# brson/synth2

Measured on AMD Instinct MI355X. Metric: voice-samples/sec (mono) at 64k voices per GPU, 48 kHz, 1024-frame buffers, higher is better.
Workload: dtype f32

## Files before the change

include/s2r.h:

```cpp
#ifndef S2R_H
#define S2R_H
#include <stddef.h>
#include <stdint.h>

#ifdef __cplusplus
extern "C" {
#endif

#define S2R_ABI_VERSION 4

typedef enum {
    S2R_OK = 0,
    S2R_ERR_INVALID = -1,
    S2R_ERR_NO_DEVICE = -2,
    S2R_ERR_HIP = -3,
    S2R_ERR_PATCH_SYNTAX = -4,
    S2R_ERR_PATCH_RANGE = -5,
    S2R_ERR_TOO_MANY_FRAMES = -6,
    S2R_ERR_OFFSET_OVERFLOW = -7,
    S2R_ERR_OUT_OF_MEMORY = -8
} s2r_status;

typedef enum { S2R_OSC_SQUARE = 0, S2R_OSC_SAW = 1, S2R_OSC_TRIANGLE = 2, S2R_OSC_SINE = 3,
               S2R_OSC_DPW_SAW = 4, S2R_OSC_DPW_SQUARE = 5, S2R_OSC_DPW_TRIANGLE = 6 } s2r_osc_kind;
// ... 189 lines not shown
uint32_t s2r_shard_voices(const s2r_synth *s);
uint32_t s2r_block_voices(const s2r_synth *s);
uint32_t s2r_device_count(const s2r_synth *s);
uint64_t s2r_double_release_count(const s2r_synth *s);
int s2r_set_low_latency(s2r_synth *s, int enabled);
int s2r_low_latency_active(const s2r_synth *s);
#define S2R_EXCHANGE_HANDLE_BYTES 64
int s2r_exchange_create(s2r_synth *s, uint32_t n_ranks, void *handle_out, size_t handle_bytes);
int s2r_exchange_attach(s2r_synth *s, uint32_t rank, uint32_t n_ranks, const void *handle, size_t handle_bytes);
int s2r_set_resident(s2r_synth *s, int enabled);
int s2r_resident_active(const s2r_synth *s);
int s2r_quiesce(s2r_synth *s);
int s2r_set_timing(s2r_synth *s, int enabled);
int s2r_set_flat_shortcut(s2r_synth *s, int enabled);
int s2r_set_coeff_stream(s2r_synth *s, int enabled);
float s2r_last_render_ms(s2r_synth *s);
const char *s2r_last_error(const s2r_synth *s);
const char *s2r_status_string(int status);


#define S2R_STREAM_CHARS_PER_SAMPLE 18u
#define S2R_STREAM_FRAMES 4096u
#define S2R_STREAM_RATE_HZ 32000u
size_t s2r_stream_frame_json(const float *samples, size_t n, char *out, size_t cap);

int s2r_parse_patch_text(const char *text, size_t len, s2r_patch *out, char *err_buf, size_t err_cap);

float s2r_voice_pan(float pan, float key_spread, uint8_t note);
void s2r_pan_gains(float p, float *gl, float *gr);

// ... 22 lines not shown
```

synth2_amd/csrc/s2r_device.h:

```cpp
#pragma once
#include <hip/hip_runtime_api.h>
#include <stdint.h>
#include "s2r.h"

#define S2R_VF_STARTED 1u
#define S2R_VF_RELEASED 2u

struct S2rEnv {
    float A;
    float D;
    float S;
    float R;
    float sus_off;
    float slope_att;
    float slope_dec;
    float slope_rel;
};

struct S2rVoiceArrays {
    float *pitch;
    uint32_t *offset;
    uint32_t *release;
    uint32_t *flags;
    float *phase;
// ... 81 lines not shown
    uint32_t super_frames;
    S2rVoiceArrays v;
    float *block_partials;
    float *direct_out;
    int32_t direct_stereo;
    S2rDone done;
    float *per_voice;
    const float *sin_table;
    const float *noise_tab;
    S2rTabRef tab;
    const S2rTimedEvent *tev;
    int32_t *voice_ev_head;
    unsigned long long *stamps;
    unsigned long long *timeline;
    uint32_t tl_slot;
    const S2rBankEntry *bank;
    uint32_t bank_size;
    const uint32_t *ov_heads_counter;
    uint32_t ov_heads_target;
    uint32_t *ov_render_counter;
    uint32_t *ov_fail;
    const S2rTimedEvent *tev_src;
    S2rTimedEvent *tev_copy;
    const uint32_t *slices;
    uint32_t *arrive;
    uint32_t arrive_target;
    S2rMixTail mt;
};

struct S2rVoiceEvent {
    uint32_t voice;
    uint32_t flags;
    float pitch;
    uint32_t seed;
};
#define S2R_EV_RESTART 1u
#define S2R_EV_RELEASE 2u
#define S2R_EV_PROGRAM_SHIFT 16

struct S2rTimedEvent {
    uint32_t voice;
    uint32_t frame;
    uint32_t flags;
// ... 198 lines not shown
```

synth2_amd/csrc/s2r_host.cpp:

```cpp
#include <hip/hip_runtime.h>
#include <algorithm>
#include <cmath>
#include <cstdarg>
#include <cstdio>
#include <cstdlib>
#include <cstring>
#include <ctime>
#include <atomic>
#include <memory>
#include <new>
#include <string>
#include <vector>

#include "s2r.h"
#include "s2r_device.h"
#include "s2r_math.h"
#include "s2r_patch.h"
#include "s2r_post.h"
#include "s2r_rules.h"
#include "s2r_voices.h"

namespace {

constexpr int kEventSlots = 4;
// ... 218 lines not shown
    float *pan_partials = nullptr;
    std::vector<hipEvent_t> pan_ev;
    size_t pan_ev_used = 0;
    float pan_mix_ms = -1.0f;
    char *bus_gains_host = nullptr, *bus_gains_dev = nullptr;
    hipEvent_t bus_gains_sent = nullptr;
    float *bus_partials = nullptr;
    float *bus_out = nullptr, *bus_out_dev = nullptr;
    float bus_mix_ms = -1.0f;
    bool bus_dev_ramped = false;
    S2rPostChain post;
    float pitch_table[256];
    hipEvent_t t0 = nullptr, t1 = nullptr;
    bool timing = false, timed = false, no_flat_shortcut = false;
    uint64_t double_release = 0;
    s2r_voice_log_fn voice_log = nullptr;
    void *voice_log_user = nullptr;
    bool broken = false;
    std::string err = "";
};


namespace {

int set_err(s2r_synth *s, int code, const char *fmt, ...) {
    if (s) {
        char buf[512];
        va_list ap; va_start(ap, fmt); vsnprintf(buf, sizeof buf, fmt, ap); va_end(ap);
        s->err = buf;
    }
// ... 293 lines not shown
    p.sr = (float)sample_rate;
    p.rcp_sr = 1.0f / p.sr;
    p.fast_div_sr = (fast_div_rate(sample_rate) && s->bank[0].lpf_freq >= 0x1p-30f && s->bank[0].lpf_freq <= 0x1p30f) ? 1 : 0;
    p.no_flat_shortcut = s->no_flat_shortcut ? 1 : 0;
    p.frames = (uint32_t)frames;
    p.n_voices = s->shard_voices;
    p.frames_stride = partials_stride(s->cfg.max_frames);
    p.v = s->v;
    p.block_partials = s->block_partials;
    p.per_voice = nullptr;
    p.sin_table = s->sin_dev;
    { static const bool off = [] { const char *e = std::getenv("S2R_NOISE_TAB"); return e && e[0] == '0'; }();
      p.noise_tab = off ? nullptr : s->noise_dev; }
    p.bank = s->bank_dev;
    p.bank_size = (uint32_t)s->bank.size();
    return p;
}

int ensure_bank(s2r_synth *s, uint32_t sample_rate, hipStream_t stream, bool *bank_kernel_out) {
    bool bank_kernel = s->bank.size() > 1;
    for (const s2r_patch &pt : s->bank) if (pt.osc_kind > S2R_OSC_SINE) bank_kernel = true;
    if (bank_kernel && (s->bank_dirty || s->bank_rate != sample_rate)) {
        std::vector<S2rBankEntry> host(s->bank.size());
        std::vector<S2rTabBuild> builds(s->bank.size());
        size_t tab_floats = 0;
        const float srf = (float)sample_rate;
        for (size_t k = 0; k < s->bank.size(); k++) {
            const s2r_patch &pt = s->bank[k];
            S2rBankEntry &e = host[k];
            std::memset(&e, 0, sizeof e);
// ... 1048 lines not shown
    if (s->voice_mem) (void)hipFree(s->voice_mem);
    if (s->bank_dev) (void)hipFree(s->bank_dev);
    if (s->os_buf) (void)hipFree(s->os_buf);
    if (s->os_taps) (void)hipFree(s->os_taps);
    if (s->block_partials) (void)hipFree(s->block_partials);
    if (s->out_dev) (void)hipFree(s->out_dev);
    if (s->out_host) (void)hipHostFree(s->out_host);
    if (s->done_host) (void)hipHostFree(s->done_host);
    if (s->done_counter) (void)hipFree(s->done_counter);
    for (int k = 0; k < 2; k++) {
        if (s->ring_host[k]) (void)hipHostFree(s->ring_host[k]);
        if (s->ring_done[k]) (void)hipEventDestroy(s->ring_done[k]);
    }
    if (s->sin_dev) (void)hipFree(s->sin_dev);
    if (s->noise_dev) (void)hipFree(s->noise_dev);
    if (s->res_cmd_vram && s->res_cmd) (void)hipFree(s->res_cmd);
    if (s->res_host) (void)hipHostFree(s->res_host);
    if (s->res_gran) (void)hipHostFree(s->res_gran);
    if (s->per_voice_dev) (void)hipFree(s->per_voice_dev);
    if (s->gains_host) (void)hipHostFree(s->gains_host);
    if (s->gains_dev) (void)hipFree(s->gains_dev);
    if (s->gains_sent) (void)hipEventDestroy(s->gains_sent);
    if (s->pan_rows) (void)hipFree(s->pan_rows);
    if (s->pan_partials) (void)hipFree(s->pan_partials);
    if (s->bus_gains_host) (void)hipHostFree(s->bus_gains_host);
    if (s->bus_gains_dev) (void)hipFree(s->bus_gains_dev);
    if (s->bus_gains_sent) (void)hipEventDestroy(s->bus_gains_sent);
    if (s->bus_partials) (void)hipFree(s->bus_partials);
    if (s->bus_out) (void)hipHostFree(s->bus_out);
    s->post.release();
// ... 183 lines not shown
    }
    CREATE_HIP(hipEventCreate(&s->t0));
    CREATE_HIP(hipEventCreate(&s->t1));
    {
        float table[1024];
        build_sin_table(table);
        if (crc32_bytes(table, sizeof table) != kSinTableCrc) {
            fprintf(stderr, "libs2r: regenerated SIN_TABLE does not match the reference table (CRC mismatch)\n");
            release_all(s);
            return S2R_ERR_INVALID;
        }
        CREATE_HIP(hipMalloc((void **)&s->sin_dev, sizeof table));
        CREATE_HIP(hipMemcpy(s->sin_dev, table, sizeof table, hipMemcpyHostToDevice));
        CREATE_HIP(hipMalloc((void **)&s->noise_dev, 65536 * sizeof(float)));
        CREATE_HIP(s2r_launch_noise_table(s->noise_dev, s->stream));
    }
    CREATE_HIP(hipStreamSynchronize(s->stream));
#undef CREATE_HIP
    *out = s;
    return S2R_OK;
}


int s2r_create(const s2r_config *cfg, s2r_synth **out) {
    if (!cfg || !out || cfg->struct_size != sizeof(s2r_config)) return S2R_ERR_INVALID;
    *out = nullptr;
    if (cfg->n_devices <= 1) {
        s2r_config one = *cfg;
        if (cfg->n_devices == 1) one.device = cfg->devices[0];
        one.n_devices = 0;
// ... 1038 lines not shown
}

uint32_t s2r_shard_voices(const s2r_synth *s) { return s ? s->shard_voices : 0; }
uint32_t s2r_block_voices(const s2r_synth *s) { return s ? s->block_voices : 0; }
uint32_t s2r_device_count(const s2r_synth *s) { return s ? (s->kids.empty() ? 1u : (uint32_t)s->kids.size()) : 0; }
uint64_t s2r_double_release_count(const s2r_synth *s) { return s ? s->double_release : 0; }

int s2r_set_flat_shortcut(s2r_synth *s, int enabled) {
    if (!s) return S2R_ERR_INVALID;
    S2R_QUIESCE(s);
    s->no_flat_shortcut = enabled == 0;
    for (s2r_synth *kid : s->kids) kid->no_flat_shortcut = s->no_flat_shortcut;
    return S2R_OK;
}

int s2r_set_coeff_stream(s2r_synth *s, int enabled) {
    if (!s) return S2R_ERR_INVALID;
    S2R_QUIESCE(s);
    s->use_tab = enabled != 0;
    s->use_arg_events = enabled != 2 && enabled != 4;
    s->bank_dirty = true;
    for (s2r_synth *kid : s->kids) { kid->use_tab = s->use_tab; kid->use_arg_events = s->use_arg_events; kid->bank_dirty = true; }
    return S2R_OK;
}

int s2r_set_low_latency(s2r_synth *s, int enabled) {
    if (!s) return S2R_ERR_INVALID;
    if (s->parent || !s->kids.empty()) return set_err(s, S2R_ERR_INVALID, "s2r_set_low_latency takes a single-device handle");
    S2R_QUIESCE(s);
    if (enabled && !s->res_host) {
// ... 211 lines not shown
```

synth2_amd/csrc/s2r_kern_common.h:

```cpp
#pragma once
#include <hip/hip_runtime.h>
#include <type_traits>
#include "s2r_device.h"
#include "s2r_math.h"

namespace {

__constant__ uint64_t c_exp2f_table[S2R_EXP2F_N] = S2R_EXP2F_TABLE_INIT;

constexpr int kChunk = 16;
constexpr uint32_t kSuperMax = 256;
constexpr uint32_t kSuperWhole = 1024;
constexpr int kP = 4;
constexpr uint32_t kTileRow = 68;

typedef float f4 __attribute__((ext_vector_type(4)));
typedef int i4 __attribute__((ext_vector_type(4)));
typedef unsigned u4 __attribute__((ext_vector_type(4)));
typedef unsigned short us4 __attribute__((ext_vector_type(4)));
typedef double d4 __attribute__((ext_vector_type(4)));
typedef unsigned long long ul4 __attribute__((ext_vector_type(4)));

__device__ __forceinline__ f4 vfma(f4 a, f4 b, f4 c) { return __builtin_elementwise_fma(a, b, c); }
__device__ __forceinline__ d4 vfma(d4 a, d4 b, d4 c) { return __builtin_elementwise_fma(a, b, c); }
// ... 703 lines not shown
        out[j] = __builtin_fmaf((s2 - s1) / 1.0f, s.tv[j] - (float)s.i1[j], s1);
    }
    return out;
}
template <bool FMV>
__device__ __forceinline__ f4 sine_quad(f4 x, f4 period, double rcp_period, const float *sSin) {
    SineQuad s = sine_quad_issue<FMV>(x, period, rcp_period, sSin);
    return sine_quad_finish(s);
}

typedef float fp2 __attribute__((ext_vector_type(2)));
__device__ __forceinline__ f4 pk_add4(f4 a, f4 b) {
    fp2 lo, hi;
    asm("v_pk_add_f32 %0, %1, %2" : "=v"(lo) : "v"(a.xy), "v"(b.xy));
    asm("v_pk_add_f32 %0, %1, %2" : "=v"(hi) : "v"(a.zw), "v"(b.zw));
    return (f4){lo.x, lo.y, hi.x, hi.y};
}

__device__ __forceinline__ void combine_groups(const S2rRenderParams &p, const S2rDone &done, const float *sWbuf, uint32_t n_groups, uint32_t super_frames,
                                               uint32_t n_sc, uint32_t sc0, float *bp_sc, uint32_t tid, uint32_t n_threads,
                                               unsigned long long *granules = nullptr, uint32_t granule_tag = 0u, bool wt = false) {
    for (uint32_t f = 4u * tid; f < n_sc; f += 4u * n_threads) {
        const float *row = sWbuf + f;
        f4 acc;
        {
            const f4 v0 = *reinterpret_cast<const f4 *>(row), v1 = *reinterpret_cast<const f4 *>(row + super_frames),
                     v2 = *reinterpret_cast<const f4 *>(row + 2u * super_frames), v3 = *reinterpret_cast<const f4 *>(row + 3u * super_frames);
            acc = pk_add4(pk_add4(pk_add4(v0, v1), v2), v3);
        }
        for (uint32_t g = 4u; g < n_groups; g += 4u) {
// ... 291 lines not shown
            ctl.mt.final_done = S2rDone{pl.final_flag + sel, s_cmd[3], nullptr};
            ctl.mt.final_stereo = stereo;
        } else {
            ctl.mt.out = o;
            ctl.mt.stereo = stereo;
            ctl.mt.done = S2rDone{pl.done_flag + sel, s_cmd[3], pl.done_counter + sel};
            if (s_cmd[12] != 0u && pl.granules != nullptr) { ctl.mt.granules = pl.granules; ctl.mt.granule_tag = s_cmd[3]; }
        }
        }
        if (frames != 0u && frames <= a.p.frames) fill(ctl);
        __syncthreads();
    }
    if (blockIdx.x == 0u && tid == 0u) __hip_atomic_store(pl.exited, pl.launch_id, __ATOMIC_RELAXED, __HIP_MEMORY_SCOPE_SYSTEM);
}

template <int OSC, int SRC, int FILT = 0, bool FMV = false, int NZ = 0, bool AFLAT = false>
__device__ __forceinline__ void chunk_fast(const S2rRenderParams &p, VoiceRegs &r, const EnvRun &ea, const EnvRun &em,
                                           const FlatCache &fc, const OscK &k, uint32_t o_chunk, const float *tab,
                                           const uint64_t *sT, const float *sSin, bool live, uint32_t tile_m0,
                                           float *pv_dst, const FiltCoef *fcoef = nullptr, Filt2 *f2 = nullptr) {
    constexpr bool SMALL = NZ >= 1, ALIGNED = NZ == 2;
    tile_set_base(tile_m0);
    f4 xq[4], bq[4], gq[4], pq[4], iq[4];
    if (SRC == 1) {
        const uint32_t plane = p.tab.plane;
#pragma unroll
        for (int q = 0; q < 4; ++q) {
            xq[q] = load_f4u(tab + 4 * q);
            if (FILT != 0) { bq[q] = load_f4u(tab + plane + 4 * q); gq[q] = load_f4u(tab + 2u * plane + 4 * q); }
            if (FMV) pq[q] = load_f4u(tab + p.tab.fm_plane * plane + 4 * q);
        }
    }
    const double rcp_period = (OSC == S2R_OSC_SINE && !FMV) ? s2r_rcp_f64(k.period) : 0.0;
    r.last = live ? r.last : 0.0f;
    const float ea_slope = live ? ea.s0 : 0.0f, ea_base = live ? ea.s1 : 0.0f, ea_y0 = live ? ea.s2 : 0.0f;
    const float xc0 = live ? fc.xc : 1.0f;
    f4 amp[4], nz[4];
    const float t_chunk = (float)o_chunk;
    const uint32_t o_lo = o_chunk & 0xffffu;
    uint32_t o01 = pk_add_u16(o_lo | (o_lo << 16), 0x00010000u), o23 = pk_add_u16(o01, 0x00020002u);
    const uint32_t seed_pair = (r.seed_rot & 0xffffu) | (r.seed_rot << 16);
    f4 t_small = splat(t_chunk) + (f4){0.0f, 1.0f, 2.0f, 3.0f};
    f4 nzt[4];
    if (ALIGNED) {
        const float *np = p.noise_tab + ((r.seed_rot ^ o_chunk) & 0xffffu);
#pragma unroll
        for (int q = 0; q < 4; ++q) nzt[q] = *reinterpret_cast<const f4 *>(np + 4 * q);
    }
#pragma unroll
    for (int q = 0; q < 4; ++q) {
        f4 t;
        if (ALIGNED) {
            t = t_small;
            t_small = t_small + splat(4.0f);
            nz[q] = nzt[q];
        } else if (SMALL) {
            t = t_small;
            nz[q] = hash_noise4_low16(seed_pair, o01, o23);
            t_small = t_small + splat(4.0f);
            o01 = pk_add_u16(o01, 0x00040004u); o23 = pk_add_u16(o23, 0x00040004u);
        } else {
            const u4 ou = (u4)(o_chunk + 4u * q) + (u4){0u, 1u, 2u, 3u};
            t = __builtin_convertvector(ou, f4);
            nz[q] = hash_noise4(r.seed_rot, t) + splat(p.noise_level);
        }
        if (AFLAT) amp[q] = splat(ea_slope * (t_chunk - ea_base) + ea_y0);
        else amp[q] = splat(ea_slope) * pk_add4(t, splat(-ea_base)) + splat(ea_y0);
// ... 3 lines not shown
            pq[q] = splat(p.sr) / f_osc;
            iq[q] = splat(1.0f) / pq[q];
        }
        if (SRC == 2) {
            const f4 mod = splat(em.s0) * (t - splat(em.s1)) + splat(em.s2);
            const f4 f_lpf = pow2_sleef_core4(mod * splat(p.amt_lpf)) * splat(p.lpf_freq);
            const f4 num = splat(-2.0f * 3.14159274101257324f) * f_lpf;
            const f4 arg = p.fast_div_sr ? div_const_nocheck4(num, p.sr, p.rcp_sr) : (num / splat(p.sr));
            xq[q] = expf4(arg, sT);
        }
    }
    const uint32_t livemask = live ? 0xffffffffu : 0u;
    f4 outs[4];
#pragma unroll
    for (int q = 0; q < 4; ++q) {
        f4 a0 = splat(1.0f) - xq[q];
        if (SRC == 2 && !live) a0 = splat(0.0f);
        const f4 period = FMV ? pq[q] : splat(k.period), inv_period = FMV ? iq[q] : splat(k.inv_period);
        f4 ph;
        float phc = r.phase;
#pragma unroll
        for (int j = 0; j < 4; ++j) {
            ph[j] = phc;
            phc = __builtin_amdgcn_fractf(phc + inv_period[j]);
        }
        r.phase = phc;
        const f4 x = period * ph;
        f4 osc;
        if (OSC == S2R_OSC_SAW) {
            const f4 ka = FMV ? splat(-2.0f) * inv_period : splat(k.a);
            osc = vfma(ka, x, splat(1.0f));
// ... 22 lines not shown
                if (SRC == 1) { cj.alpha = xq[q][j]; cj.beta = bq[q][j]; cj.gamma = gq[q][j]; }
                y[j] = dsp_filter_apply(FILT, cj, sv[j], *f2);
            }
        }
        f4 out = y * amp[q];
        if (FILT != 0) out = (f4)((u4)out & livemask);
        tile_store4(q, out);
        outs[q] = out;
    }
    if (pv_dst) {
#pragma unroll
        for (int q = 0; q < 4; ++q) *reinterpret_cast<f4u *>(pv_dst + 4 * q) = outs[q];
    }
}

}
```

synth2_amd/csrc/s2r_render_onepole.inc:

```
#include "s2r_kern_common.h"

namespace {

template <int OSC, bool FM, int MODE, int MAXT>
__device__ __forceinline__ void render_fill(const S2rRenderArgs &a, const FillCtl &ctl) {
    const S2rRenderParams &p = a.p;
    constexpr bool PV = MODE == 1;
    constexpr bool TEV = MODE == 2;
    const uint32_t kSuper = p.super_frames;
    __shared__ uint64_t sT[S2R_EXP2F_N];
    __shared__ __attribute__((aligned(8))) float sSin[OSC == S2R_OSC_SINE ? 2048 : 2];
    extern __shared__ __attribute__((aligned(16))) float s_dyn[];
    __shared__ uint32_t s_word;

    const uint32_t tid = threadIdx.x;
    const uint32_t lane = tid & 63u, wave = tid >> 6, n_waves = blockDim.x >> 6;
    constexpr uint32_t VW = 64;
    constexpr uint32_t GW = VW / 16;
    const uint32_t n_groups = n_waves * GW;
    float *const sW = s_dyn;
    constexpr uint32_t kTile = kChunk * kTileRow;
    const uint32_t sw_floats = s2r_sw_buffers(p.frames, kSuper) * n_groups * kSuper;
    float *const tile = s_dyn + sw_floats + wave * kTile;
    float *const wave_scratch = s_dyn + sw_floats + n_waves * kTile + wave * 64u;
    const uint32_t tile_lds = (uint32_t)__builtin_amdgcn_readfirstlane((int)(uint32_t)(uintptr_t)tile);
    const uint32_t vi = blockIdx.x * blockDim.x + tid;
#if defined(S2R_STAMPS)
    uint32_t stamp_k = 0;
    auto stamp = [&](uint32_t slot) { if (p.stamps && lane == 0 && slot < 16u) p.stamps[(size_t)(vi >> 6) * 16u + slot] = __builtin_amdgcn_s_memtime(); };
    stamp(0);
#else
    auto stamp = [&](uint32_t) {};
    uint32_t stamp_k = 0; (void)stamp_k;
#endif
    uint32_t dbg_events = 0, dbg_dense = 0, dbg_general = 0, dbg_runs = 0, dbg_runchunks = 0;
    unsigned long long dbg_t_dense = 0, dbg_t_run = 0;
    unsigned long long dbg_t_top = 0, dbg_t_sel = 0; (void)dbg_t_top; (void)dbg_t_sel;
    unsigned long long dbg_t_pick1 = 0, dbg_t_casc = 0; (void)dbg_t_pick1; (void)dbg_t_casc;
    (void)dbg_events; (void)dbg_dense; (void)dbg_general; (void)dbg_runs; (void)dbg_runchunks; (void)dbg_t_dense; (void)dbg_t_run;
// ... 116 lines not shown
    uint32_t buf = 0;

    auto reduce_chunk = [&](uint32_t f_base, uint32_t n_frames) {
        const uint32_t f = lane & 15u, grp = lane >> 4;
        __builtin_amdgcn_wave_barrier();
        if (f < n_frames) {
            const float *src = tile + f * kTileRow + grp * 16u;
            float acc = src[0];
#pragma unroll
            for (int k = 1; k < 16; ++k) acc += src[k];
            sW[(buf * n_groups + wave * GW + grp) * kSuper + f_base + f] = acc;
        }
        __builtin_amdgcn_wave_barrier();
    };

    bool w_flat = false, w_aflat = false, w_aligned = false, w_small = false;
    auto reclassify_stages = [&]() {
        w_flat = !p.no_flat_shortcut && __ballot(live && em.s0 != 0.0f) == 0ull &&
                 (!FM || __ballot(!(fc.k.period >= 0x1p-126f && fc.k.period < __builtin_inff())) == 0ull);
        w_aflat = __ballot(live && ea.s0 != 0.0f) == 0ull;
    };
    auto reclassify = [&]() {
        reclassify_stages();
        w_aligned = p.noise_tab != nullptr && __ballot(((r.offset | r.seed_rot) & 15u) != 0u) == 0ull;
        w_small = __ballot(r.offset + ctl.frames > (1u << 24)) == 0ull;
    };
    reclassify();
    stamp(1);

    auto apply_events_lane = [&](uint32_t fpos) -> bool {
        bool restarted = false, released_now = false;
        took_release = false;
        while (ev_frame == fpos) {
            const S2rTimedEvent e = ev_next;
            if (e.flags & S2R_EV_RESTART) {
// ... 48 lines not shown
    };

    auto apply_events_at = [&](uint32_t fpos) {
        if (!wave_events || __ballot(ev_frame == fpos) == 0ull) return;
        dbg_events += (uint32_t)__builtin_popcountll(__ballot(ev_frame == fpos));
        bool restarted = false;
        if (ev_frame == fpos) restarted = apply_events_lane(fpos);
        if (__ballot(restarted) != 0ull) {
            w_aligned = p.noise_tab != nullptr && __ballot(((r.offset | r.seed_rot) & 15u) != 0u) == 0ull;
            w_small = __ballot(r.offset + ctl.frames > (1u << 24)) == 0ull;
        }
        wave_events = __ballot(ev_idx >= 0) != 0ull;
        w_flat = !p.no_flat_shortcut && __ballot(live && em.s0 != 0.0f) == 0ull &&
                 (!FM || __ballot(!(fc.k.period >= 0x1p-126f && fc.k.period < __builtin_inff())) == 0ull);
        w_aflat = __ballot(live && ea.s0 != 0.0f) == 0ull;
    };

    auto end_of_release = [&](float t0) {
        if (ea.s4 == 3.0f && !(t0 < ea.s3)) { ea.s0 = 0.0f; ea.s1 = 0.0f; ea.s2 = 0.0f; ea.s3 = __builtin_inff(); ea.s4 = 4.0f; }
        if (em.s4 == 3.0f && !(t0 < em.s3)) { em.s0 = 0.0f; em.s1 = 0.0f; em.s2 = 0.0f; em.s3 = __builtin_inff(); em.s4 = 4.0f; }
        if (ea.s4 == 2.0f && !(t0 < ea.s3)) { const bool rel = t0 < r.end_a;
            ea.s0 = rel ? p.amp.slope_rel : 0.0f; ea.s1 = rel ? r.ro_a : 0.0f; ea.s2 = rel ? p.amp.S : 0.0f;
            ea.s3 = rel ? r.end_a : __builtin_inff(); ea.s4 = rel ? 3.0f : 4.0f; }
        if (em.s4 == 2.0f && !(t0 < em.s3)) { const bool rel = t0 < r.end_m;
            em.s0 = rel ? p.mod.slope_rel : 0.0f; em.s1 = rel ? r.ro_m : 0.0f; em.s2 = rel ? p.mod.S : 0.0f;
            em.s3 = rel ? r.end_m : __builtin_inff(); em.s4 = rel ? 3.0f : 4.0f; }
    };

    const uint32_t rf = lane & 15u, rgrp = lane >> 4;
    const float *const tsrc = tile + rf * kTileRow + rgrp * 16u;
// ... 153 lines not shown
                    bool flat = false, tab_ok = false, offs_small = false;
                    if (run) {
                        run = (uint32_t)__builtin_amdgcn_readfirstlane((int)run);
                        offs_small = w_small || __ballot(o_chunk + run * kChunk > (1u << 24)) == 0ull;
                        flat = w_flat;
                        tab_ok = !flat && have_tab && offs_small;
                        if (FM && !flat && !tab_ok) run = 0;
                        if (FM && !flat && __ballot(live && !(p.sr >= r.pitch * 0x1p-115f)) != 0ull) run = 0;
                    }
                    if (run) {
                        ++dbg_runs; dbg_runchunks += run;
                        const unsigned long long dbg_tr0 = S2R_DBG_NOW();
                        dbg_t_sel += dbg_tr0 - dbg_ts0;
                        float *const sw_row = sW + (buf * n_groups + wave * GW + rgrp) * kSuper + rf;
                        const TabCur cur = tab_cursor(p.tab, em.s4, r.ro_m > p.mod.sus_off, r.release_u, live);
                        auto run_chunks = [&](auto src_tag, auto nz_tag, auto aflat_tag) {
                            constexpr int SRC = decltype(src_tag)::value;
                            constexpr int NZ = decltype(nz_tag)::value;
                            constexpr bool AFLAT = decltype(aflat_tag)::value;
                            for (uint32_t i = 0; i < run; ++i) {
                                const uint32_t f0 = c16 + i * kChunk;
                                *pend_dst = tsum();
                                float *pvd = (PV && in_range) ? p.per_voice + pv_base + sc0 + f0 : nullptr;
                                const uint32_t oc = o_chunk + i * kChunk;
                                const float *tp = p.tab.base + (ptrdiff_t)(cur.idx + (int32_t)(oc & cur.mask));
                                chunk_fast<OSC, SRC, 0, (FM && SRC == 1), NZ, AFLAT>(p, r, ea, em, fc, FM ? fc.k : k_const, oc, tp, sT, sSin, live,
                                                                              tile_lds, pvd);
                                __builtin_amdgcn_wave_barrier();
                                pend_dst = sw_row + f0;
                            }
                        };
                        const bool small = p.noise_level == 0.0f && offs_small;
                        const bool aligned = small && w_aligned && ((sc0 + c16) & 15u) == 0u;
                        const bool aflat = aligned && w_aflat;
                        using T = std::true_type; using F = std::false_type;
                        using N0 = std::integral_constant<int, 0>; using N1 = std::integral_constant<int, 1>; using N2 = std::integral_constant<int, 2>;
                        if (tab_ok) {
                            if (aflat) run_chunks(N1{}, N2{}, T{});
                            else if (aligned) run_chunks(N1{}, N2{}, F{});
                            else if (small) run_chunks(N1{}, N1{}, F{});
                            else run_chunks(N1{}, N0{}, F{});
                        } else if (flat) {
                            if (aflat) run_chunks(N0{}, N2{}, T{});
                            else if (aligned) run_chunks(N0{}, N2{}, F{});
                            else if (small) run_chunks(N0{}, N1{}, F{});
                            else run_chunks(N0{}, N0{}, F{});
                        } else if (!FM) {
                            if (aligned) run_chunks(N2{}, N2{}, F{});
                            else if (small) run_chunks(N2{}, N1{}, F{});
                            else run_chunks(N2{}, N0{}, F{});
                        }
                        c16 += (run - 1u) * kChunk;
                        dbg_t_run += S2R_DBG_NOW() - dbg_tr0;
                        continue;
                    }
                }
                flush_pending();
                ++dbg_general;
                for (uint32_t g = c16; g < c16 + kChunk; g += kP) {
                    FrameCF4 cf; OscK4 kf;
                    closed_form_x4<OSC, FM>(p, r, ea, em, thr_min, fc, fcc, r.offset + sc0 + g, sT, cf, kf);
                    f4 out4;
#pragma unroll
                    for (int j = 0; j < kP; ++j) {
                        FrameCF c1; c1.amp = cf.amp[j]; c1.xc = cf.xc[j]; c1.nz = cf.nz[j];
// ... 42 lines not shown
        p.v.offset[vi] = (!ev_dirty && o > 0xffffffffu - ctl.frames) ? 0xffffffffu : o + ctl.frames;
        p.v.phase[vi] = r.phase;
        p.v.lpf_last[vi] = r.last;
        if (ev_dirty) {
            p.v.pitch[vi] = r.pitch;
            p.v.release[vi] = r.release_u;
            p.v.flags[vi] = S2R_VF_STARTED | (r.released ? S2R_VF_RELEASED : 0u);
            p.v.seed[vi] = seed_now;
            if (ev_restart) {
                p.v.fx1[vi] = 0.0f; p.v.fx2[vi] = 0.0f; p.v.fy1[vi] = 0.0f; p.v.fy2[vi] = 0.0f;
                p.v.osc_z[vi] = s2r_u2f(S2R_OSC_Z_NONE);
                p.v.program[vi] = program_now;
            }
        }
    }
    if (p.direct_out && ctl.granules == nullptr) signal_done(ctl.done, 1u);
    if (ctl.ov_render_counter != nullptr) ov_signal(ctl.ov_render_counter);
#if defined(S2R_STAMPS)
    if (p.stamps && lane == 0) p.stamps[(size_t)(vi >> 6) * 16u + 8u] = __builtin_amdgcn_s_memrealtime();
    if (ctl.fused) fused_tail(p, ctl, sW, &s_word, p.stamps ? p.stamps + (size_t)(vi >> 6) * 16u : nullptr);
#else
    if (ctl.fused) fused_tail(p, ctl, sW, &s_word);
#endif
#if defined(S2R_STAMPS)
    if (p.stamps && lane == 0) { unsigned long long *d = p.stamps + (size_t)(vi >> 6) * 16u; d[11] = dbg_events; d[12] = (unsigned long long)dbg_dense | ((dbg_t_pick1 & 0x3fffffull) << 20) | ((dbg_t_casc & 0x3fffffull) << 42); d[13] = (dbg_t_top << 32) | (dbg_t_sel & 0xffffffffull); d[14] = dbg_runs;
        d[10] = ((unsigned long long)dbg_runchunks << 48) | ((dbg_t_dense & 0xffffffull) << 24) | (dbg_t_run & 0xffffffull); }
#endif
    stamp(15);
    tl_mark(p.timeline, p.tl_slot, 1);
}

template <int OSC, bool FM, int MODE, int MAXT>
__global__ void __launch_bounds__(MAXT, (MAXT == 256 ? 2 : 1)) s2r_render_kernel(const S2rRenderArgs a) {
    const FillCtl ctl = fill_ctl_from_args(a);
    render_fill<OSC, FM, MODE, MAXT>(a, ctl);
}

template <int OSC, bool FM>
__global__ void __launch_bounds__(256, 1) s2r_resident_kernel(const S2rRenderArgs a, const S2rResident rs) {
    __shared__ uint32_t s_cmd[S2R_RES_CMD_WORDS];
    const uint32_t tid = threadIdx.x, lane = tid & 63u;
    uint32_t last = rs.first_seq - 1u;
    for (;;) {
        if (tid < 64u) {
            const unsigned long long t0 = __builtin_amdgcn_s_memrealtime();
            uint32_t polls = 0;
            for (;;) {
                uint32_t w = 0u;
                if (lane < S2R_RES_CMD_WORDS) w = __hip_atomic_load(rs.cmd + lane, __ATOMIC_RELAXED, __HIP_MEMORY_SCOPE_SYSTEM);
                const uint32_t s_first = (uint32_t)__builtin_amdgcn_readlane((int)w, 0), s_last = (uint32_t)__builtin_amdgcn_readlane((int)w, 31);
// ... 26 lines not shown
}

template <int OSC, bool FM>
__global__ void __launch_bounds__(256, 1) s2r_pool_kernel(const S2rRenderArgs a, const S2rPool pl) {
    pool_loop(a, pl, [&](const FillCtl &ctl) __attribute__((always_inline)) { render_fill<OSC, FM, 2, 256>(a, ctl); });
}

template <int OSC, bool FM, int MODE>
hipError_t launch_mode(const S2rRenderArgs &a0, uint32_t block_voices, hipStream_t stream) {
    static thread_local S2rRenderArgs a;
    a = a0;
    S2rRenderParams &p = a.p;
    const uint32_t grid = (p.n_voices + block_voices - 1) / block_voices;
    const uint32_t n_waves = block_voices / 64, n_groups = n_waves * 4;
    p.super_frames = s2r_pick_super_frames(n_groups, grid, p.frames);
    const size_t lds = sizeof(float) * ((size_t)s2r_sw_buffers(p.frames, p.super_frames) * n_groups * p.super_frames + (size_t)n_waves * (kChunk * kTileRow + 64));
    if (lds > 65536) {
        static thread_local size_t told256 = 0, told1024 = 0;
        if (block_voices <= 256 && told256 < lds) {
            const hipError_t e = hipFuncSetAttribute((const void *)s2r_render_kernel<OSC, FM, MODE, 256>, hipFuncAttributeMaxDynamicSharedMemorySize, (int)lds);
            if (e != hipSuccess) return e;
            told256 = lds;
        } else if (block_voices > 256 && told1024 < lds) {
            const hipError_t e = hipFuncSetAttribute((const void *)s2r_render_kernel<OSC, FM, MODE, 1024>, hipFuncAttributeMaxDynamicSharedMemorySize, (int)lds);
            if (e != hipSuccess) return e;
            told1024 = lds;
        }
    }
    if (block_voices <= 256) hipLaunchKernelGGL((s2r_render_kernel<OSC, FM, MODE, 256>), dim3(grid), dim3(block_voices), lds, stream, a);
    else hipLaunchKernelGGL((s2r_render_kernel<OSC, FM, MODE, 1024>), dim3(grid), dim3(block_voices), lds, stream, a);
    return hipGetLastError();
}

template <int OSC, bool FM>
hipError_t launch_resident(const S2rRenderArgs &a0, const S2rResident &rs, uint32_t block_voices, hipStream_t stream) {
    static thread_local S2rRenderArgs a;
    a = a0;
    S2rRenderParams &p = a.p;
    if (block_voices > 256u || p.n_voices > block_voices || p.direct_out == nullptr || p.per_voice != nullptr || p.tev != nullptr) return hipErrorInvalidValue;
    const uint32_t n_waves = block_voices / 64, n_groups = n_waves * 4;
    p.super_frames = s2r_pick_super_frames(n_groups, 1u, p.frames);
    const size_t lds = sizeof(float) * ((size_t)s2r_sw_buffers(p.frames, p.super_frames) * n_groups * p.super_frames + (size_t)n_waves * (kChunk * kTileRow + 64));
    if (lds > 65536) {
        static thread_local size_t told = 0;
        if (told < lds) {
            const hipError_t e = hipFuncSetAttribute((const void *)s2r_resident_kernel<OSC, FM>, hipFuncAttributeMaxDynamicSharedMemorySize, (int)lds);
            if (e != hipSuccess) return e;
            told = lds;
        }
    }
    hipLaunchKernelGGL((s2r_resident_kernel<OSC, FM>), dim3(1), dim3(block_voices), lds, stream, a, rs);
    return hipGetLastError();
}

template <int OSC, bool FM>
hipError_t launch_pool(const S2rRenderArgs &a0, const S2rPool &pl, uint32_t block_voices, hipStream_t stream) {
    static thread_local S2rRenderArgs a;
    a = a0;
    S2rRenderParams &p = a.p;
    if (block_voices > 256u || p.per_voice != nullptr || p.direct_out != nullptr) return hipErrorInvalidValue;
    const uint32_t grid = (p.n_voices + block_voices - 1) / block_voices;
    const uint32_t n_waves = block_voices / 64, n_groups = n_waves * 4;
    p.super_frames = s2r_pick_super_frames(n_groups, grid, p.frames);
    const size_t lds = sizeof(float) * ((size_t)s2r_sw_buffers(p.frames, p.super_frames) * n_groups * p.super_frames + (size_t)n_waves * (kChunk * kTileRow + 64));
    if (lds > 65536) {
        static thread_local size_t told = 0;
        if (told < lds) {
            const hipError_t e = hipFuncSetAttribute((const void *)s2r_pool_kernel<OSC, FM>, hipFuncAttributeMaxDynamicSharedMemorySize, (int)lds);
            if (e != hipSuccess) return e;
            told = lds;
        }
    }
    hipLaunchKernelGGL((s2r_pool_kernel<OSC, FM>), dim3(grid), dim3(block_voices), lds, stream, a, pl);
    return hipGetLastError();
}

}

// ... 22 lines not shown
```

synth2_amd/synth.py:

```python
import ctypes as C
import os

import numpy as np

from . import build as _build

OSC_SQUARE, OSC_SAW, OSC_TRIANGLE, OSC_SINE = 0, 1, 2, 3
OSC_DPW_SAW, OSC_DPW_SQUARE, OSC_DPW_TRIANGLE = 4, 5, 6

S2R_OK = 0
S2R_ERR_INVALID = -1
S2R_ERR_NO_DEVICE = -2
S2R_ERR_HIP = -3
S2R_ERR_PATCH_SYNTAX = -4
S2R_ERR_PATCH_RANGE = -5
S2R_ERR_TOO_MANY_FRAMES = -6
S2R_ERR_OFFSET_OVERFLOW = -7
S2R_ERR_OUT_OF_MEMORY = -8
MAX_BUSES = 8
MAX_IR_TAPS = 65536
MAX_DELAY_FRAMES = 262144
IR_SEGMENT = 256
METER_BLOCK = 256
LIMITER_MAX_LOOKAHEAD = 1024
# ... 183 lines not shown
        "s2r_set_noise_seed": (C.c_int, [H, C.c_uint32, C.c_uint32]),
        "s2r_shard_voices": (C.c_uint32, [H]),
        "s2r_block_voices": (C.c_uint32, [H]),
        "s2r_device_count": (C.c_uint32, [H]),
        "s2r_double_release_count": (C.c_uint64, [H]),
        "s2r_set_timing": (C.c_int, [H, C.c_int]),
        "s2r_set_low_latency": (C.c_int, [H, C.c_int]),
        "s2r_low_latency_active": (C.c_int, [H]),
        "s2r_set_resident": (C.c_int, [H, C.c_int]),
        "s2r_resident_active": (C.c_int, [H]),
        "s2r_quiesce": (C.c_int, [H]),
        "s2r_exchange_create": (C.c_int, [H, C.c_uint32, C.c_void_p, C.c_size_t]),
        "s2r_exchange_attach": (C.c_int, [H, C.c_uint32, C.c_uint32, C.c_void_p, C.c_size_t]),
        "s2r_set_flat_shortcut": (C.c_int, [H, C.c_int]),
        "s2r_set_coeff_stream": (C.c_int, [H, C.c_int]),
        "s2r_last_render_ms": (C.c_float, [H]),
        "s2r_last_error": (C.c_char_p, [H]),
        "s2r_parse_patch_text": (C.c_int, [C.c_char_p, C.c_size_t, C.POINTER(Patch), C.c_char_p, C.c_size_t]),
        "s2r_voice_pool_create": (H, [C.c_uint32]),
        "s2r_voice_pool_destroy": (None, [H]),
        "s2r_voice_pool_note_on": (C.c_uint32, [H, C.c_uint8, C.c_float]),
        "s2r_voice_pool_note_off": (C.c_int64, [H, C.c_uint8]),
        "s2r_voice_pool_advance": (None, [H, C.c_uint64]),
        "s2r_voice_pool_next_voice": (C.c_uint32, [H]),
        "s2r_voice_pool_set_threads": (None, [H, C.c_uint32, C.c_size_t]),
        "s2r_voice_pool_resolve": (C.c_uint32, [H, C.c_void_p, C.c_size_t, C.c_uint32, C.c_void_p]),
        "s2r_voice_pool_query": (C.c_int, [H, C.c_uint32, C.POINTER(VoiceState)]),
    }
    for name, (res, args) in sig.items():
        if _build.AB_LIB and not hasattr(L, name):
# ... 524 lines not shown

    def import_state(self, arr):
        arr = np.ascontiguousarray(arr, dtype=VOICE_STATE_DTYPE)
        assert arr.size == self.shard_voices
        self._check(self.L.s2r_import_state(self.h, arr.ctypes.data))

    def set_noise_seed(self, voice_index, seed):
        self._check(self.L.s2r_set_noise_seed(self.h, voice_index, seed))

    def set_flat_shortcut(self, enabled=True):
        self._check(self.L.s2r_set_flat_shortcut(self.h, 1 if enabled else 0))

    def set_coeff_stream(self, enabled=True):
        self._check(self.L.s2r_set_coeff_stream(self.h, int(enabled)))

    def set_low_latency(self, enabled=True):
        self._check(self.L.s2r_set_low_latency(self.h, 1 if enabled else 0))

    @property
    def low_latency_active(self):
        return bool(self.L.s2r_low_latency_active(self.h))

    def set_resident(self, enabled=True):
        self._check(self.L.s2r_set_resident(self.h, 1 if enabled else 0))

    @property
    def resident_active(self):
        return bool(self.L.s2r_resident_active(self.h))

    def quiesce(self):
# ... 24 lines not shown
```

Baseline: 1652 billion.

## Share per-frame oscillator, envelope and noise window across wave-uniform voices

Adds a per-wave check for whether all 64 lanes share the same table cursor, offset, noise seed and envelope state. When they do, and the run is long enough, the lanes work together to compute the wavetable sample, 1-x, amplitude ramp and noise for the run once into an LDS window, and each lane's chunk then reads those planes. This removes per-lane redundant table, noise and envelope work. The cost is extra LDS per wave, which can lower occupancy, plus classification ballots and a global atomic counter. The path is on by default for 256-thread non-FM kernels.

New measurement: 1707 billion (median of 6 runs). 3.3% higher.

```diff
diff --git a/include/s2r.h b/include/s2r.h
--- a/include/s2r.h
+++ b/include/s2r.h
@@ -227,6 +227,8 @@
 int s2r_set_timing(s2r_synth *s, int enabled);
 int s2r_set_flat_shortcut(s2r_synth *s, int enabled);
 int s2r_set_coeff_stream(s2r_synth *s, int enabled);
+int s2r_set_uniform_window(s2r_synth *s, int enabled);
+int s2r_uniform_window_chunks(s2r_synth *s, uint64_t *chunks);
 float s2r_last_render_ms(s2r_synth *s);
 const char *s2r_last_error(const s2r_synth *s);
 const char *s2r_status_string(int status);
diff --git a/synth2_amd/csrc/s2r_device.h b/synth2_amd/csrc/s2r_device.h
--- a/synth2_amd/csrc/s2r_device.h
+++ b/synth2_amd/csrc/s2r_device.h
@@ -119,6 +119,7 @@
     unsigned long long *stamps;
     unsigned long long *timeline;
     uint32_t tl_slot;
+    uint32_t uw_frames;
     const S2rBankEntry *bank;
     uint32_t bank_size;
     const uint32_t *ov_heads_counter;
@@ -131,7 +132,11 @@
     uint32_t *arrive;
     uint32_t arrive_target;
     S2rMixTail mt;
-};
+    uint32_t *uw_count;
+};
+#define S2R_UW_FRAMES 1024u
+#define S2R_UW_PLANES 4u
+#define S2R_UW_MIN_RUN 3u
 
 struct S2rVoiceEvent {
     uint32_t voice;
diff --git a/synth2_amd/csrc/s2r_host.cpp b/synth2_amd/csrc/s2r_host.cpp
--- a/synth2_amd/csrc/s2r_host.cpp
+++ b/synth2_amd/csrc/s2r_host.cpp
@@ -256,6 +256,8 @@
     hipEvent_t t0 = nullptr, t1 = nullptr;
     bool timing = false, timed = false, no_flat_shortcut = false;
     uint64_t double_release = 0;
+    bool uniform_window = true;
+    uint32_t *uw_count_dev = nullptr;
     s2r_voice_log_fn voice_log = nullptr;
     void *voice_log_user = nullptr;
     bool broken = false;
@@ -579,6 +581,7 @@
       p.noise_tab = off ? nullptr : s->noise_dev; }
     p.bank = s->bank_dev;
     p.bank_size = (uint32_t)s->bank.size();
+    p.uw_count = s->uniform_window ? s->uw_count_dev : nullptr;
     return p;
 }
 
@@ -1657,6 +1660,7 @@
     }
     if (s->sin_dev) (void)hipFree(s->sin_dev);
     if (s->noise_dev) (void)hipFree(s->noise_dev);
+    if (s->uw_count_dev) (void)hipFree(s->uw_count_dev);
     if (s->res_cmd_vram && s->res_cmd) (void)hipFree(s->res_cmd);
     if (s->res_host) (void)hipHostFree(s->res_host);
     if (s->res_gran) (void)hipHostFree(s->res_gran);
@@ -1870,6 +1874,8 @@
         CREATE_HIP(hipMemcpy(s->sin_dev, table, sizeof table, hipMemcpyHostToDevice));
         CREATE_HIP(hipMalloc((void **)&s->noise_dev, 65536 * sizeof(float)));
         CREATE_HIP(s2r_launch_noise_table(s->noise_dev, s->stream));
+        CREATE_HIP(hipMalloc((void **)&s->uw_count_dev, sizeof(uint32_t)));
+        CREATE_HIP(hipMemsetAsync(s->uw_count_dev, 0, sizeof(uint32_t), s->stream));
     }
     CREATE_HIP(hipStreamSynchronize(s->stream));
 #undef CREATE_HIP
@@ -2938,6 +2944,33 @@
     return S2R_OK;
 }
 
+int s2r_set_uniform_window(s2r_synth *s, int enabled) {
+    if (!s) return S2R_ERR_INVALID;
+    S2R_QUIESCE(s);
+    s->uniform_window = enabled != 0;
+    for (s2r_synth *kid : s->kids) kid->uniform_window = s->uniform_window;
+    return S2R_OK;
+}
+
+int s2r_uniform_window_chunks(s2r_synth *s, uint64_t *chunks) {
+    if (!s || !chunks) return S2R_ERR_INVALID;
+    S2R_QUIESCE(s);
+    uint64_t total = 0;
+    auto one = [&](s2r_synth *h) -> int {
+        if (!h->uw_count_dev) return S2R_OK;
+        uint32_t n = 0;
+        S2R_HIP(s, hipSetDevice(h->device));
+        S2R_HIP(s, hipDeviceSynchronize());
+        S2R_HIP(s, hipMemcpy(&n, h->uw_count_dev, sizeof n, hipMemcpyDeviceToHost));
+        total += n;
+        return S2R_OK;
+    };
+    if (s->kids.empty()) { S2R_TRY(one(s)); }
+    else for (s2r_synth *kid : s->kids) { S2R_TRY(one(kid)); }
+    *chunks = total;
+    return S2R_OK;
+}
+
 int s2r_set_coeff_stream(s2r_synth *s, int enabled) {
     if (!s) return S2R_ERR_INVALID;
     S2R_QUIESCE(s);
diff --git a/synth2_amd/csrc/s2r_kern_common.h b/synth2_amd/csrc/s2r_kern_common.h
--- a/synth2_amd/csrc/s2r_kern_common.h
+++ b/synth2_amd/csrc/s2r_kern_common.h
@@ -741,6 +741,12 @@
     fp2 lo, hi;
     asm("v_pk_add_f32 %0, %1, %2" : "=v"(lo) : "v"(a.xy), "v"(b.xy));
     asm("v_pk_add_f32 %0, %1, %2" : "=v"(hi) : "v"(a.zw), "v"(b.zw));
+    return (f4){lo.x, lo.y, hi.x, hi.y};
+}
+__device__ __forceinline__ f4 pk_sub4(f4 a, f4 b) {
+    fp2 lo, hi;
+    asm("v_pk_add_f32 %0, %1, %2 neg_lo:[0,1] neg_hi:[0,1]" : "=v"(lo) : "v"(a.xy), "v"(b.xy));
+    asm("v_pk_add_f32 %0, %1, %2 neg_lo:[0,1] neg_hi:[0,1]" : "=v"(hi) : "v"(a.zw), "v"(b.zw));
     return (f4){lo.x, lo.y, hi.x, hi.y};
 }
 
@@ -1062,15 +1068,26 @@
     if (blockIdx.x == 0u && tid == 0u) __hip_atomic_store(pl.exited, pl.launch_id, __ATOMIC_RELAXED, __HIP_MEMORY_SCOPE_SYSTEM);
 }
 
-template <int OSC, int SRC, int FILT = 0, bool FMV = false, int NZ = 0, bool AFLAT = false>
+template <int OSC, int SRC, int FILT = 0, bool FMV = false, int NZ = 0, bool AFLAT = false, bool UW = false>
 __device__ __forceinline__ void chunk_fast(const S2rRenderParams &p, VoiceRegs &r, const EnvRun &ea, const EnvRun &em,
                                            const FlatCache &fc, const OscK &k, uint32_t o_chunk, const float *tab,
                                            const uint64_t *sT, const float *sSin, bool live, uint32_t tile_m0,
-                                           float *pv_dst, const FiltCoef *fcoef = nullptr, Filt2 *f2 = nullptr) {
+                                           float *pv_dst, const FiltCoef *fcoef = nullptr, Filt2 *f2 = nullptr,
+                                           const float *win = nullptr) {
     constexpr bool SMALL = NZ >= 1, ALIGNED = NZ == 2;
+    static_assert(!UW || (SRC == 1 && FILT == 0 && !FMV && NZ == 2 && !AFLAT), "the uniform window replaces one variant only");
     tile_set_base(tile_m0);
     f4 xq[4], bq[4], gq[4], pq[4], iq[4];
-    if (SRC == 1) {
+    f4 a0w[4], ampw[4], nzw[4];
+    if (UW) {
+#pragma unroll
+        for (int q = 0; q < 4; ++q) {
+            xq[q] = *reinterpret_cast<const f4 *>(win + 4 * q);
+            a0w[q] = *reinterpret_cast<const f4 *>(win + S2R_UW_FRAMES + 4 * q);
+            ampw[q] = *reinterpret_cast<const f4 *>(win + 2u * S2R_UW_FRAMES + 4 * q);
+            nzw[q] = *reinterpret_cast<const f4 *>(win + 3u * S2R_UW_FRAMES + 4 * q);
+        }
+    } else if (SRC == 1) {
         const uint32_t plane = p.tab.plane;
 #pragma unroll
         for (int q = 0; q < 4; ++q) {
@@ -1090,7 +1107,7 @@
     const uint32_t seed_pair = (r.seed_rot & 0xffffu) | (r.seed_rot << 16);
     f4 t_small = splat(t_chunk) + (f4){0.0f, 1.0f, 2.0f, 3.0f};
     f4 nzt[4];
-    if (ALIGNED) {
+    if (ALIGNED && !UW) {
         const float *np = p.noise_tab + ((r.seed_rot ^ o_chunk) & 0xffffu);
 #pragma unroll
         for (int q = 0; q < 4; ++q) nzt[q] = *reinterpret_cast<const f4 *>(np + 4 * q);
@@ -1098,7 +1115,10 @@
 #pragma unroll
     for (int q = 0; q < 4; ++q) {
         f4 t;
-        if (ALIGNED) {
+        if (UW) {
+            nz[q] = nzw[q]; amp[q] = ampw[q];
+            continue;
+        } else if (ALIGNED) {
             t = t_small;
             t_small = t_small + splat(4.0f);
             nz[q] = nzt[q];
@@ -1132,7 +1152,7 @@
     f4 outs[4];
 #pragma unroll
     for (int q = 0; q < 4; ++q) {
-        f4 a0 = splat(1.0f) - xq[q];
+        f4 a0 = UW ? a0w[q] : SRC == 1 ? pk_sub4(splat(1.0f), xq[q]) : splat(1.0f) - xq[q];
         if (SRC == 2 && !live) a0 = splat(0.0f);
         const f4 period = FMV ? pq[q] : splat(k.period), inv_period = FMV ? iq[q] : splat(k.inv_period);
         f4 ph;
@@ -1185,4 +1205,26 @@
     }
 }
 
-}
+__device__ __forceinline__ void uw_fill(const S2rRenderParams &p, const EnvRun &ea, uint32_t seed_rot, uint32_t o_run, uint32_t run,
+                                        const float *tab_run, float *win, uint32_t lane) {
+    const uint32_t n_quads = 4u * run;
+    for (uint32_t q0 = 0; q0 < n_quads; q0 += 64u) {
+        const uint32_t Q = q0 + lane;
+        if (Q < n_quads) {
+            const uint32_t o = o_run + 4u * Q;
+            const f4 x = load_f4u(tab_run + 4u * Q);
+            const f4 a0 = pk_sub4(splat(1.0f), x);
+            const f4 t = splat((float)o) + (f4){0.0f, 1.0f, 2.0f, 3.0f};
+            const f4 amp = splat(ea.s0) * pk_add4(t, splat(-ea.s1)) + splat(ea.s2);
+            const f4 nz = *reinterpret_cast<const f4 *>(p.noise_tab + ((seed_rot ^ (o & ~15u)) & 0xffffu) + (o & 15u));
+            float *w = win + 4u * Q;
+            *reinterpret_cast<f4 *>(w) = x;
+            *reinterpret_cast<f4 *>(w + S2R_UW_FRAMES) = a0;
+            *reinterpret_cast<f4 *>(w + 2u * S2R_UW_FRAMES) = amp;
+            *reinterpret_cast<f4 *>(w + 3u * S2R_UW_FRAMES) = nz;
+        }
+    }
+    __builtin_amdgcn_wave_barrier();
+}
+
+}
diff --git a/synth2_amd/csrc/s2r_render_onepole.inc b/synth2_amd/csrc/s2r_render_onepole.inc
--- a/synth2_amd/csrc/s2r_render_onepole.inc
+++ b/synth2_amd/csrc/s2r_render_onepole.inc
@@ -2,7 +2,7 @@
 
 namespace {
 
-template <int OSC, bool FM, int MODE, int MAXT>
+template <int OSC, bool FM, int MODE, int MAXT, bool UWK = false>
 __device__ __forceinline__ void render_fill(const S2rRenderArgs &a, const FillCtl &ctl) {
     const S2rRenderParams &p = a.p;
     constexpr bool PV = MODE == 1;
@@ -22,7 +22,8 @@
     constexpr uint32_t kTile = kChunk * kTileRow;
     const uint32_t sw_floats = s2r_sw_buffers(p.frames, kSuper) * n_groups * kSuper;
     float *const tile = s_dyn + sw_floats + wave * kTile;
-    float *const wave_scratch = s_dyn + sw_floats + n_waves * kTile + wave * 64u;
+    float *const wave_scratch = s_dyn + sw_floats + n_waves * kTile + wave * (64u + (UWK ? S2R_UW_PLANES * p.uw_frames : 0u));
+    uint32_t uw_chunks = 0;
     const uint32_t tile_lds = (uint32_t)__builtin_amdgcn_readfirstlane((int)(uint32_t)(uintptr_t)tile);
     const uint32_t vi = blockIdx.x * blockDim.x + tid;
 #if defined(S2R_STAMPS)
@@ -169,11 +170,20 @@
         __builtin_amdgcn_wave_barrier();
     };
 
-    bool w_flat = false, w_aflat = false, w_aligned = false, w_small = false;
+    bool w_flat = false, w_aflat = false, w_aligned = false, w_small = false, w_uni = false;
+    auto classify_uniform = [&]() {
+        if (!(UWK && !FM) || p.uw_frames == 0u) return;
+        const TabCur c = tab_cursor(p.tab, em.s4, r.ro_m > p.mod.sus_off, r.release_u, live);
+        auto differs = [](uint32_t v) { return v != (uint32_t)__builtin_amdgcn_readfirstlane((int)v); };
+        const bool odd = !live || c.mask != 0xffffffffu || differs((uint32_t)c.idx) || differs(r.offset) || differs(r.seed_rot) ||
+                         differs(s2r_f2u(ea.s0)) || differs(s2r_f2u(ea.s1)) || differs(s2r_f2u(ea.s2)) || differs(s2r_f2u(em.s4));
+        w_uni = __ballot(odd) == 0ull;
+    };
     auto reclassify_stages = [&]() {
         w_flat = !p.no_flat_shortcut && __ballot(live && em.s0 != 0.0f) == 0ull &&
                  (!FM || __ballot(!(fc.k.period >= 0x1p-126f && fc.k.period < __builtin_inff())) == 0ull);
         w_aflat = __ballot(live && ea.s0 != 0.0f) == 0ull;
+        classify_uniform();
     };
     auto reclassify = [&]() {
         reclassify_stages();
@@ -252,6 +262,7 @@
         w_flat = !p.no_flat_shortcut && __ballot(live && em.s0 != 0.0f) == 0ull &&
                  (!FM || __ballot(!(fc.k.period >= 0x1p-126f && fc.k.period < __builtin_inff())) == 0ull);
         w_aflat = __ballot(live && ea.s0 != 0.0f) == 0ull;
+        classify_uniform();
     };
 
     auto end_of_release = [&](float t0) {
@@ -435,18 +446,24 @@
                         dbg_t_sel += dbg_tr0 - dbg_ts0;
                         float *const sw_row = sW + (buf * n_groups + wave * GW + rgrp) * kSuper + rf;
                         const TabCur cur = tab_cursor(p.tab, em.s4, r.ro_m > p.mod.sus_off, r.release_u, live);
-                        auto run_chunks = [&](auto src_tag, auto nz_tag, auto aflat_tag) {
+                        auto run_chunks = [&](auto src_tag, auto nz_tag, auto aflat_tag, auto uw_tag) {
                             constexpr int SRC = decltype(src_tag)::value;
                             constexpr int NZ = decltype(nz_tag)::value;
                             constexpr bool AFLAT = decltype(aflat_tag)::value;
+                            constexpr bool UW = decltype(uw_tag)::value;
+                            if (UW) {
+                                const uint32_t o_run = (uint32_t)__builtin_amdgcn_readfirstlane((int)o_chunk);
+                                uw_fill(p, ea, r.seed_rot, o_run, run, p.tab.base + (ptrdiff_t)(cur.idx + (int32_t)o_chunk), wave_scratch + 64u, lane);
+                                uw_chunks += run;
+                            }
                             for (uint32_t i = 0; i < run; ++i) {
                                 const uint32_t f0 = c16 + i * kChunk;
                                 *pend_dst = tsum();
                                 float *pvd = (PV && in_range) ? p.per_voice + pv_base + sc0 + f0 : nullptr;
                                 const uint32_t oc = o_chunk + i * kChunk;
                                 const float *tp = p.tab.base + (ptrdiff_t)(cur.idx + (int32_t)(oc & cur.mask));
-                                chunk_fast<OSC, SRC, 0, (FM && SRC == 1), NZ, AFLAT>(p, r, ea, em, fc, FM ? fc.k : k_const, oc, tp, sT, sSin, live,
-                                                                              tile_lds, pvd);
+                                chunk_fast<OSC, SRC, 0, (FM && SRC == 1), NZ, AFLAT, UW>(p, r, ea, em, fc, FM ? fc.k : k_const, oc, tp, sT, sSin, live,
+                                                                              tile_lds, pvd, nullptr, nullptr, wave_scratch + 64u + i * kChunk);
                                 __builtin_amdgcn_wave_barrier();
                                 pend_dst = sw_row + f0;
                             }
@@ -456,20 +473,23 @@
                         const bool aflat = aligned && w_aflat;
                         using T = std::true_type; using F = std::false_type;
                         using N0 = std::integral_constant<int, 0>; using N1 = std::integral_constant<int, 1>; using N2 = std::integral_constant<int, 2>;
+                        using UWon = std::integral_constant<bool, UWK && !FM>;
+                        const bool uw = UWon::value && w_uni && run >= S2R_UW_MIN_RUN;
                         if (tab_ok) {
-                            if (aflat) run_chunks(N1{}, N2{}, T{});
-                            else if (aligned) run_chunks(N1{}, N2{}, F{});
-                            else if (small) run_chunks(N1{}, N1{}, F{});
-                            else run_chunks(N1{}, N0{}, F{});
+                            if (aflat) run_chunks(N1{}, N2{}, T{}, F{});
+                            else if (aligned && uw) run_chunks(N1{}, N2{}, F{}, UWon{});
+                            else if (aligned) run_chunks(N1{}, N2{}, F{}, F{});
+                            else if (small) run_chunks(N1{}, N1{}, F{}, F{});
+                            else run_chunks(N1{}, N0{}, F{}, F{});
                         } else if (flat) {
-                            if (aflat) run_chunks(N0{}, N2{}, T{});
-                            else if (aligned) run_chunks(N0{}, N2{}, F{});
-                            else if (small) run_chunks(N0{}, N1{}, F{});
-                            else run_chunks(N0{}, N0{}, F{});
+                            if (aflat) run_chunks(N0{}, N2{}, T{}, F{});
+                            else if (aligned) run_chunks(N0{}, N2{}, F{}, F{});
+                            else if (small) run_chunks(N0{}, N1{}, F{}, F{});
+                            else run_chunks(N0{}, N0{}, F{}, F{});
                         } else if (!FM) {
-                            if (aligned) run_chunks(N2{}, N2{}, F{});
-                            else if (small) run_chunks(N2{}, N1{}, F{});
-                            else run_chunks(N2{}, N0{}, F{});
+                            if (aligned) run_chunks(N2{}, N2{}, F{}, F{});
+                            else if (small) run_chunks(N2{}, N1{}, F{}, F{});
+                            else run_chunks(N2{}, N0{}, F{}, F{});
                         }
                         c16 += (run - 1u) * kChunk;
                         dbg_t_run += S2R_DBG_NOW() - dbg_tr0;
@@ -542,6 +562,7 @@
             }
         }
     }
+    if (UWK && uw_chunks != 0u && lane == 0u) __hip_atomic_fetch_add(p.uw_count, uw_chunks, __ATOMIC_RELAXED, __HIP_MEMORY_SCOPE_AGENT);
     if (p.direct_out && ctl.granules == nullptr) signal_done(ctl.done, 1u);
     if (ctl.ov_render_counter != nullptr) ov_signal(ctl.ov_render_counter);
 #if defined(S2R_STAMPS)
@@ -561,7 +582,7 @@
 template <int OSC, bool FM, int MODE, int MAXT>
 __global__ void __launch_bounds__(MAXT, (MAXT == 256 ? 2 : 1)) s2r_render_kernel(const S2rRenderArgs a) {
     const FillCtl ctl = fill_ctl_from_args(a);
-    render_fill<OSC, FM, MODE, MAXT>(a, ctl);
+    render_fill<OSC, FM, MODE, MAXT, MAXT == 256>(a, ctl);
 }
 
 template <int OSC, bool FM>
@@ -618,7 +639,12 @@
     const uint32_t grid = (p.n_voices + block_voices - 1) / block_voices;
     const uint32_t n_waves = block_voices / 64, n_groups = n_waves * 4;
     p.super_frames = s2r_pick_super_frames(n_groups, grid, p.frames);
-    const size_t lds = sizeof(float) * ((size_t)s2r_sw_buffers(p.frames, p.super_frames) * n_groups * p.super_frames + (size_t)n_waves * (kChunk * kTileRow + 64));
+    size_t lds = sizeof(float) * ((size_t)s2r_sw_buffers(p.frames, p.super_frames) * n_groups * p.super_frames + (size_t)n_waves * (kChunk * kTileRow + 64));
+    p.uw_frames = 0u;
+    if (p.uw_count != nullptr && !FM && block_voices <= 256 && p.super_frames == kSuperWhole && s2r_sw_buffers(p.frames, p.super_frames) == 1u) {
+        const size_t with_uw = lds + sizeof(float) * (size_t)n_waves * S2R_UW_PLANES * S2R_UW_FRAMES;
+        if (with_uw + 8192u + 8u * S2R_EXP2F_N + 64u <= 160u * 1024u) { lds = with_uw; p.uw_frames = S2R_UW_FRAMES; }
+    }
     if (lds > 65536) {
         static thread_local size_t told256 = 0, told1024 = 0;
         if (block_voices <= 256 && told256 < lds) {
@@ -644,6 +670,7 @@
     if (block_voices > 256u || p.n_voices > block_voices || p.direct_out == nullptr || p.per_voice != nullptr || p.tev != nullptr) return hipErrorInvalidValue;
     const uint32_t n_waves = block_voices / 64, n_groups = n_waves * 4;
     p.super_frames = s2r_pick_super_frames(n_groups, 1u, p.frames);
+    p.uw_frames = 0u;
     const size_t lds = sizeof(float) * ((size_t)s2r_sw_buffers(p.frames, p.super_frames) * n_groups * p.super_frames + (size_t)n_waves * (kChunk * kTileRow + 64));
     if (lds > 65536) {
         static thread_local size_t told = 0;
@@ -666,6 +693,7 @@
     const uint32_t grid = (p.n_voices + block_voices - 1) / block_voices;
     const uint32_t n_waves = block_voices / 64, n_groups = n_waves * 4;
     p.super_frames = s2r_pick_super_frames(n_groups, grid, p.frames);
+    p.uw_frames = 0u;
     const size_t lds = sizeof(float) * ((size_t)s2r_sw_buffers(p.frames, p.super_frames) * n_groups * p.super_frames + (size_t)n_waves * (kChunk * kTileRow + 64));
     if (lds > 65536) {
         static thread_local size_t told = 0;
diff --git a/synth2_amd/synth.py b/synth2_amd/synth.py
--- a/synth2_amd/synth.py
+++ b/synth2_amd/synth.py
@@ -221,6 +221,8 @@
         "s2r_exchange_attach": (C.c_int, [H, C.c_uint32, C.c_uint32, C.c_void_p, C.c_size_t]),
         "s2r_set_flat_shortcut": (C.c_int, [H, C.c_int]),
         "s2r_set_coeff_stream": (C.c_int, [H, C.c_int]),
+        "s2r_set_uniform_window": (C.c_int, [H, C.c_int]),
+        "s2r_uniform_window_chunks": (C.c_int, [H, C.POINTER(C.c_uint64)]),
         "s2r_last_render_ms": (C.c_float, [H]),
         "s2r_last_error": (C.c_char_p, [H]),
         "s2r_parse_patch_text": (C.c_int, [C.c_char_p, C.c_size_t, C.POINTER(Patch), C.c_char_p, C.c_size_t]),
@@ -775,6 +777,14 @@
     def set_coeff_stream(self, enabled=True):
         self._check(self.L.s2r_set_coeff_stream(self.h, int(enabled)))
 
+    def set_uniform_window(self, enabled=True):
+        self._check(self.L.s2r_set_uniform_window(self.h, 1 if enabled else 0))
+
+    def uniform_window_chunks(self):
+        n = C.c_uint64(0)
+        self._check(self.L.s2r_uniform_window_chunks(self.h, C.byref(n)))
+        return int(n.value)
+
     def set_low_latency(self, enabled=True):
         self._check(self.L.s2r_set_low_latency(self.h, 1 if enabled else 0))
 
```
